# TtesseractT/Synthetic-Audio-Detection

Measured on AMD Instinct MI355X. Metric: 4s@32kHz segments/sec end-to-end (mel+ResNet+ensemble), 1/2/4/8 MI355X, higher is better.
Workload: dtype bf16; 1 GPU; end-to-end inference: B int16 4 s segments resident in HBM -> mel front end -> ResNet-18@512x512 -> 6 binary heads -> merge (+RCCL all-gather of logits); heads=6, distinct_backbones=1, micro_batch=2048, parallelism=dp1, frontend_overlapped=True

## Files before the change

synthetic-audio-detection_amd/csrc/halo256rs2.hip:

```cpp
#include "common.hpp"
#include "igemm.hpp"
#include "kernels.hpp"
#include "rwconv.hpp"

namespace sad {

namespace h44 {
constexpr int NW = 8, TC = 2;
constexpr int PW = 17, PITCH = PW * 128;
constexpr int NR[4] = {17, 17, 16, 16};
constexpr int NCV[4] = {17, 16, 17, 16};
constexpr int NP[4] = {37, 37, 34, 34};
constexpr int OFF[4] = {0, 37 * 1024, 74 * 1024, 108 * 1024};
constexpr int SMEM = 142 * 1024;
constexpr int BAD = 0x7FFFFFF0;
constexpr uint64_t KEY = 0x7929284ef1797ull;
static_assert(SMEM <= 160 * 1024, "LDS budget");
static_assert(16 * PITCH < 65536, "fragment row offsets are ds_read immediates");
constexpr int TPL[9] = {0, 0, 0, 0, 1, 1, 2, 2, 3};
constexpr int TRO[9] = {0, 0, 1, 1, 0, 1, 0, 0, 0};
constexpr int TCO[9] = {0, 1, 0, 1, 0, 0, 0, 1, 0};
constexpr int TAP[9] = {0, 2, 6, 8, 1, 7, 3, 5, 4};
constexpr int SCH[9][3] = {
    {1 | 3 << 3, 2 | 1 << 3, -1}, {1 | 4 << 3, 2 | 2 << 3, -1}, {2 | 3 << 3, 3 | 0 << 3, -1},
    {2 | 4 << 3, 3 | 1 << 3, -1}, {0 | 4 | 0 << 3, 3 | 2 << 3, -1}, {0 | 4 | 1 << 3, 3 | 3 << 3, -1},
    {0 | 4 | 2 << 3, 1 | 4 | 0 << 3, 3 | 4 << 3}, {0 | 4 | 3 << 3, 1 | 4 | 1 << 3, -1},
    {0 | 4 | 4 << 3, 1 | 4 | 2 << 3, 2 | 4 | 0 << 3}};
constexpr uint64_t pack_sch(int e) {
  uint64_t v = 0;
  for (int T = 0; T < 9; ++T) v |= (uint64_t)(SCH[T][e] < 0 ? 0x7F : SCH[T][e]) << (7 * T);
  return v;
}
constexpr uint64_t SCHP0 = pack_sch(0), SCHP1 = pack_sch(1), SCHP2 = pack_sch(2);
constexpr uint64_t pack_step() {
  uint64_t v = 0;
  for (int T = 0; T < 9; ++T) v |= (uint64_t)(TPL[T] | TRO[T] << 2 | TCO[T] << 3) << (4 * T);
  return v;
}
constexpr uint64_t STEPP = pack_step();
constexpr uint64_t pack_tap() {
  uint64_t v = 0;
  for (int T = 0; T < 8; ++T) v |= (uint64_t)TAP[T + 1] << (4 * T);
  return v;
}
constexpr uint64_t TAPP = pack_tap();
}

__device__ __forceinline__ int h44_key(int x) { return (int)((h44::KEY >> (3 * x)) & 7); }

typedef unsigned int h44_v4 __attribute__((ext_vector_type(4)));
typedef __bf16 h44_bf2 __attribute__((ext_vector_type(2)));
typedef float h44_f2 __attribute__((ext_vector_type(2)));
template <typename E = u16>
__device__ __forceinline__ uint32_t h44_pk(float lo, float hi) {
  if constexpr (is_f16_v<E>) return pk_f16(lo, hi);
  return __builtin_bit_cast(uint32_t, __builtin_convertvector((h44_f2){lo, hi}, h44_bf2));
}
__device__ __forceinline__ uint32_t h44_relu2(uint32_t x) {
  uint32_t r;
  asm("v_pk_max_i16 %0, %1, 0" : "=v"(r) : "v"(x));
  return r;
}

template <int BC, bool X3, typename E = u16>
__global__ __launch_bounds__(512, 1) void halo256rs2_kernel(BlockConvArgs a) {
  static_assert(!is_f16_v<E> || !X3, "fp16 has no split form");
  f16_kernel_entry<E>();
  using namespace h44;
  constexpr int NCG = BC / 32, NPG = NW / NCG, TP = 16 / NPG;
  static_assert(NCG * NPG == NW, "wave split");
  extern __shared__ __attribute__((aligned(16))) char smem[];
  const int tid = threadIdx.x, lane = tid & 63;
  const int wave = __builtin_amdgcn_readfirstlane(tid >> 6);
  const int fr = lane & 15, fg = lane >> 4;
  const int n_tc = a.Cout / BC;
  const int w = xcd_remap(blockIdx.x, gridDim.x);
  const int tc = w % n_tc;
  const int gp = gridDim.x / n_tc, wi = w / n_tc;
  const int tiles_x = a.Wo / 16, tiles_img = tiles_x * (a.Ho / 16);
  const int tiles_p = a.N * tiles_img;
  const int tp_begin = (int)((int64_t)wi * tiles_p / gp), tp_end = (int)((int64_t)(wi + 1) * tiles_p / gp);
  if (tp_begin >= tp_end) return;
  const int cgrp = wave % NCG, pgrp = wave / NCG;
  const int cw = tc * BC + cgrp * 16 * TC;
  const int r0w = pgrp * TP;
  const int ab = a.ablate;

  const int cinb = a.Cin * 2;
  const int nch = cinb / 128;
  const __amdgpu_buffer_rsrc_t r0 =
      __builtin_amdgcn_make_buffer_rsrc((void*)a.in0, (short)0, (int)a.in0_bytes, 0x00020000);
  const __amdgpu_buffer_rsrc_t rw =
      __builtin_amdgcn_make_buffer_rsrc((void*)a.wt, (short)0, (int)a.wt_bytes, 0x00020000);
  const int ps = (int)a.in0_pstride * 2;
  const unsigned lds0 = (unsigned)(uintptr_t)(__attribute__((address_space(3))) char*)smem;

  const int wrow = a.wt_ld * 2;
  const int wlane = (cw + fr) * wrow + fg * 16;
  auto load_w = [&](int kb, h44_v4 (&wv)[TC][2]) __attribute__((always_inline)) {
#pragma unroll
    for (int i = 0; i < TC; ++i)
#pragma unroll
      for (int h = 0; h < 2; ++h)
        wv[i][h] = __builtin_amdgcn_raw_buffer_load_b128(rw, wlane + i * 16 * wrow + h * 64,
                                                         __builtin_amdgcn_readfirstlane(kb), 0);
  };

  struct TileO {
    int b, iy0, ix0;
    bool ok;
  };
  auto tile_o = [&](int t) __attribute__((always_inline)) {
    const int tt = __builtin_amdgcn_readfirstlane(t);
    const int b = tt / tiles_img, rem = tt - b * tiles_img;
    const int ty = rem / tiles_x;
    return TileO{b, 32 * ty - 1, 32 * (rem - ty * tiles_x) - 1, tt < tp_end};
  };
  auto issue = [&](int P, const TileO& to, int c, int k) __attribute__((always_inline)) {
    const int q = wave + NW * k;
    const int np = P < 2 ? 37 : 34, nr = P < 2 ? 17 : 16, ncv = (P & 1) ? 16 : 17;
    if (q >= np || !to.ok) return;
    int ln;
    asm volatile("v_mov_b32 %0, %1" : "=v"(ln) : "v"(lane));
    const int u = 8 * q + (ln >> 3);
    const int r = (u * 3856) >> 16;
    const int x = u - PW * r;
    const int iy = to.iy0 + 2 * r + (P >> 1), ix = to.ix0 + 2 * x + (P & 1);
    const bool ok = r < nr && x < ncv && iy >= 0 && ix >= 0;
    const int off = ((to.b * a.H + iy) * a.W + ix) * ps + c * 128 + (((ln & 7) ^ h44_key(x)) << 4);
    const int poff = P == 0 ? OFF[0] : P == 1 ? OFF[1] : P == 2 ? OFF[2] : OFF[3];
    dma16_m0(r0, ok ? off : BAD, lds0 + poff + q * 1024);
  };

  {
    const TileO t0 = tile_o(tp_begin);
    for (int k = 0; k < 5; ++k) issue(0, t0, 0, k);
    for (int k = 0; k < 3; ++k) issue(1, t0, 0, k);
    issue(2, t0, 0, 0);
  }
  f32x4 biasv[TC];
#pragma unroll
  for (int i = 0; i < TC; ++i) biasv[i] = *(const f32x4*)(a.bias + cw + i * 16 + fg * 4);
  h44_v4 wcur[TC][2], wnxt[TC][2];
  load_w(0, wnxt);
  f32x4 acc[TC][TP];
#pragma unroll
  for (int i = 0; i < TC; ++i)
#pragma unroll
    for (int j = 0; j < TP; ++j) acc[i][j] = biasv[i];
  auto take_w = [&]() __attribute__((always_inline)) {
#pragma unroll
    for (int i = 0; i < TC; ++i)
#pragma unroll
      for (int h = 0; h < 2; ++h) wcur[i][h] = wnxt[i][h];
  };

  int lofs[2][2];
#pragma unroll
  for (int co = 0; co < 2; ++co)
#pragma unroll
    for (int h = 0; h < 2; ++h)
      lofs[co][h] = r0w * PITCH + (fr + co) * 128 + (((4 * h + fg) ^ h44_key(fr + co)) << 4);

  auto step = [&](int pbase, int co) __attribute__((always_inline)) {
    auto half = [&](auto hc) __attribute__((always_inline)) {
      constexpr int h = decltype(hc)::value;
      constexpr int NM = X3 && h == 0 ? 2 : 1;
      const char* pb = smem + pbase + (co ? lofs[1][h] : lofs[0][h]);
      uint4 bf[TP];
#pragma unroll
      for (int j = 0; j < TP; ++j) bf[j] = *(const uint4*)(pb + j * PITCH);
#pragma unroll
      for (int j = 0; j < TP; ++j)
#pragma unroll
        for (int m = 0; m < NM; ++m)
#pragma unroll
          for (int i = 0; i < TC; ++i)
            mfma_chunk<E>(__builtin_bit_cast(uint4, wcur[i][X3 ? m : h]), bf[j], acc[i][j]);
      __builtin_amdgcn_sched_group_barrier(0x100, 4, 0);
#pragma unroll
      for (int j = 0; j < TP - 4; ++j) {
        __builtin_amdgcn_sched_group_barrier(0x008, NM * TC, 0);
        __builtin_amdgcn_sched_group_barrier(0x100, 1, 0);
      }
      __builtin_amdgcn_sched_group_barrier(0x008, 4 * NM * TC, 0);
    };
    half(std::integral_constant<int, 0>{});
    half(std::integral_constant<int, 1>{});
  };

  auto epilogue = [&](int t) __attribute__((always_inline)) {
    const int b = t / tiles_img, rem = t - b * tiles_img;
    const int oy0 = (rem / tiles_x) * 16, ox0 = (rem - (rem / tiles_x) * tiles_x) * 16;
    u16* __restrict__ out = (u16*)a.out;
#pragma unroll
    for (int j = 0; j < TP; j += 2) {
      const int64_t px = (int64_t)(b * a.Ho + oy0 + r0w + j + (fg & 1)) * a.Wo + ox0 + fr;
#pragma unroll
      for (int i = 0; i < TC; ++i) {
        if constexpr (X3) {
          float v[2][4];
#pragma unroll
          for (int r = 0; r < 4; ++r) {
            v[0][r] = a.relu ? fmaxf(acc[i][j][r], 0.f) : acc[i][j][r];
            v[1][r] = a.relu ? fmaxf(acc[i][j + 1][r], 0.f) : acc[i][j + 1][r];
          }
          uint32_t qh[4], ql[4];
#pragma unroll
          for (int e = 0; e < 4; ++e) {
            const float x0 = v[e >> 1][2 * (e & 1)], x1 = v[e >> 1][2 * (e & 1) + 1];
            qh[e] = h44_pk(x0, x1);
            ql[e] = h44_pk(x0 - __uint_as_float(qh[e] << 16), x1 - __uint_as_float(qh[e] & 0xFFFF0000u));
          }
#pragma unroll
          for (int e = 0; e < 2; ++e) {
            const auto rh = __builtin_amdgcn_permlane16_swap(qh[e], qh[e + 2], false, false);
            qh[e] = rh[0];
            qh[e + 2] = rh[1];
            const auto rl = __builtin_amdgcn_permlane16_swap(ql[e], ql[e + 2], false, false);
            ql[e] = rl[0];
            ql[e + 2] = rl[1];
          }
          u16* op = out + px * a.out_pstride + 2 * cw + i * 16 + (fg >> 1) * 8;
          *(uint4*)op = make_uint4(qh[0], qh[1], qh[2], qh[3]);
          *(uint4*)(op + 32) = make_uint4(ql[0], ql[1], ql[2], ql[3]);
          continue;
        }
        const int co = cw + i * 16 + (fg >> 1) * 8;
        uint32_t q[4] = {h44_pk<E>(acc[i][j][0], acc[i][j][1]), h44_pk<E>(acc[i][j][2], acc[i][j][3]),
                         h44_pk<E>(acc[i][j + 1][0], acc[i][j + 1][1]), h44_pk<E>(acc[i][j + 1][2], acc[i][j + 1][3])};
        if (a.relu)
#pragma unroll
          for (int e = 0; e < 4; ++e) q[e] = h44_relu2(q[e]);
#pragma unroll
        for (int e = 0; e < 2; ++e) {
          const auto r = __builtin_amdgcn_permlane16_swap(q[e], q[e + 2], false, false);
          q[e] = r[0];
          q[e + 2] = r[1];
        }
        *(uint4*)(out + px * a.out_pstride + co) = make_uint4(q[0], q[1], q[2], q[3]);
      }
    }
#pragma unroll
    for (int i = 0; i < TC; ++i)
#pragma unroll
      for (int j = 0; j < TP; ++j) acc[i][j] = biasv[i];
  };

  bool post_epi = false;
  for (int t = tp_begin; t < tp_end; ++t) {
    const TileO tcur = tile_o(t), tnext = tile_o(t + 1);
    for (int c = 0; c < nch; ++c) {
      const int ncn = c + 1 < nch ? c + 1 : 0;
      const TileO& tn = c + 1 < nch ? tcur : tnext;
#pragma unroll 1
      for (int T = 0; T < 9; ++T) {
        if ((T == 0 || T == 4 || T == 6 || T == 8) && !(ab & 16)) {
          if (T == 0 && post_epi)
            asm volatile("s_waitcnt vmcnt(%0)" ::"n"((X3 ? 2 : 1) * TC * TP / 2) : "memory");
          else
            asm volatile("s_waitcnt vmcnt(0)" ::: "memory");
          post_epi = false;
          __builtin_amdgcn_s_barrier();
          asm volatile("" ::: "memory");
        }
        take_w();
        const int kbn = T < 8 ? (int)((TAPP >> (4 * T)) & 15) * cinb + c * 128 : ncn * 128;
        if (!(ab & 4)) load_w(kbn, wnxt);
        if (!(ab & 2)) {
#pragma unroll
          for (int e = 0; e < 3; ++e) {
            const uint64_t sp = e == 0 ? SCHP0 : e == 1 ? SCHP1 : SCHP2;
            const int d = (int)((sp >> (7 * T)) & 0x7F);
            if (d != 0x7F) {
              const bool nx = (d >> 2) & 1;
              issue(d & 3, nx ? tn : tcur, nx ? ncn : c, d >> 3);
            }
          }
        }
        const int sd = (int)((STEPP >> (4 * T)) & 15), pl = sd & 3;
        int co;
        asm volatile("s_lshr_b32 %0, %1, 3" : "=s"(co) : "s"(sd));
        step(1024 * (37 * pl - (pl == 3 ? 3 : 0)) + ((sd >> 2) & 1) * PITCH, co);
      }
    }
    if (!(ab & 8)) epilogue(t);
    post_epi = true;
  }
  asm volatile("s_waitcnt vmcnt(0)" ::: "memory");
}

template <int BC, bool X3, typename E = u16>
static int launch_halo256rs2_t(const BlockConvArgs& a, hipStream_t s) {
  using namespace h44;
  static bool attr = false;
  if (!attr) {
    SAD_CHECK_HIP(hipFuncSetAttribute((const void*)halo256rs2_kernel<BC, X3, E>,
                                      hipFuncAttributeMaxDynamicSharedMemorySize, SMEM));
    attr = true;
  }
  const int n_tc = a.Cout / BC;
  const int64_t tiles_p = (int64_t)a.N * (a.Ho / 16) * (a.Wo / 16);
  int64_t g = std::min<int64_t>(tiles_p * n_tc, 256);
  g = std::max<int64_t>(n_tc, g / n_tc * n_tc);
  hipLaunchKernelGGL((halo256rs2_kernel<BC, X3, E>), dim3((unsigned)g), dim3(512), SMEM, s, a);
  SAD_CHECK_HIP(hipGetLastError());
  return SAD_OK;
}

bool halo256rs2_ok(const BlockConvArgs& a) {
  return a.KH == 3 && a.KW == 3 && a.stride == 2 && a.pad == 1 && !a.in1 && !a.res && !a.st_part && !a.pool_out &&
         a.Cin % 64 == 0 && a.Cout % 128 == 0 && a.Ho % 16 == 0 && a.Wo % 16 == 0 && a.H == 2 * a.Ho &&
         a.W == 2 * a.Wo;
}

int launch_halo256rs2(const BlockConvArgs& a, hipStream_t s, bool x3, bool h16) {
  SAD_REQUIRE(!(x3 && h16), "variant 44: fp16 has no split form");
  SAD_REQUIRE(a.KH == 3 && a.KW == 3 && a.stride == 2 && a.pad == 1 && !a.in1 && !a.res && !a.st_part &&
                  !a.pool_out,
              "variant 44: 3x3/s2/p1, no shortcut / residual / pool / statistics");
  SAD_REQUIRE((a.Cin * 2) % 128 == 0 && a.Cout % 128 == 0, "variant 44: whole 128-B chunks, Cout % 128");
  SAD_REQUIRE(a.Ho % 16 == 0 && a.Wo % 16 == 0 && a.H == 2 * a.Ho && a.W == 2 * a.Wo,
              "variant 44: 16 x 16 output tiles, input exactly twice the output");
  SAD_REQUIRE(a.wt_ld >= 9 * a.Cin && (a.wt_ld * 2) % 16 == 0, "variant 44: weight rows");
  SAD_REQUIRE(a.out_pstride % 8 == 0 && a.in0_pstride % 8 == 0, "variant 44: pixel strides");
  SAD_REQUIRE(a.out != nullptr, "null output");
  SAD_REQUIRE(a.M == (int64_t)a.N * a.Ho * a.Wo, "variant 44: M = N Ho Wo");
  SAD_REQUIRE(((int64_t)a.N * a.H * a.W - 1) * a.in0_pstride * 2 + 2 * a.Cin < (1ll << 31) - 65536,
              "variant 44: input passes the 32-bit buffer range");
  if (h16)
    return a.Cout % 256 == 0 ? launch_halo256rs2_t<256, false, f16>(a, s) : launch_halo256rs2_t<128, false, f16>(a, s);
  if (x3)
    return a.Cout % 256 == 0 ? launch_halo256rs2_t<256, true>(a, s) : launch_halo256rs2_t<128, true>(a, s);
  return a.Cout % 256 == 0 ? launch_halo256rs2_t<256, false>(a, s) : launch_halo256rs2_t<128, false>(a, s);
}

}
```

synthetic-audio-detection_amd/csrc/l2s2conv.hip:

```cpp
#include "common.hpp"
#include "igemm.hpp"
#include "kernels.hpp"
#include "rwconv.hpp"

namespace sad {

namespace l2s {
constexpr int NW = 4;
constexpr int PRR = 17, PCW = 33;
constexpr int NEV = 9;
constexpr int PXB = 128;
constexpr int ROWB = PCW * PXB;
constexpr int ODDC = 17 * PXB;
constexpr int NPX = PRR * PCW;
constexpr int NDP = (NPX * PXB + 1023) / 1024;
constexpr int PATCH = NDP * 1024;
constexpr int QP = (NDP + NW - 1) / NW;
constexpr int OFF_BIAS = 2 * PATCH;
constexpr int SMEM = OFF_BIAS + 512;
constexpr int NS = 18;
constexpr int TP = 8;
constexpr int NUC = 9 * 2 * TP;
constexpr int DQ = 8;
constexpr int PDIV = 8;
constexpr int BAD = 0x7FFFFFF0;
constexpr uint64_t KEY = 0x7929284ef1797ull;
static_assert(SMEM <= 160 * 1024, "LDS budget");
static_assert(NUC / PDIV >= QP, "pieces fit the chunk's units");
static_assert(NW - 1 + NW * (QP - 2) < NDP, "only the last piece index can pass the patch");
static_assert(8 * ROWB + ODDC + 16 * PXB <= 65535, "fragment offsets are ds_read immediates");
}

__device__ __forceinline__ int l2s_key(int x) { return (int)((l2s::KEY >> (3 * x)) & 7); }

template <bool ST = false, typename E = u16>
__global__ __launch_bounds__(256, 1) void l2s2conv_kernel(BlockConvArgs a) {
  static_assert(!is_f16_v<E> || !ST, "the fused statistics are the bf16 trainer's");
  f16_kernel_entry<E>();
  using namespace l2s;
  const int ab = a.ablate;
  extern __shared__ __attribute__((aligned(16))) char smem[];
  const int tid = threadIdx.x, lane = tid & 63;
  const int wave = __builtin_amdgcn_readfirstlane(tid >> 6);
  const int fr = lane & 15, fg = lane >> 4;
  const int cw = wave * 32;
  const int w = xcd_remap(blockIdx.x, gridDim.x);
  const int tiles_x = a.Wo / 16, tiles_img = tiles_x * (a.Ho / 16);
  const int tiles_p = a.N * tiles_img;
  const int tp_begin = (int)((int64_t)w * tiles_p / gridDim.x), tp_end = (int)((int64_t)(w + 1) * tiles_p / gridDim.x);
  if (tp_begin >= tp_end) {
    if constexpr (ST) a.st_part[(int64_t)w * 256 + tid] = 0.f;
    return;
  }

  const __amdgpu_buffer_rsrc_t rx =
      __builtin_amdgcn_make_buffer_rsrc((void*)a.in0, (short)0, (int)a.in0_bytes, 0x00020000);
  const __amdgpu_buffer_rsrc_t ro =
      __builtin_amdgcn_make_buffer_rsrc((void*)a.out, (short)0, (int)a.out_bytes, 0x00020000);
  const unsigned lds0 = (unsigned)(uintptr_t)(__attribute__((address_space(3))) char*)smem;
  const int ps = (int)a.in0_pstride * 2;

  struct TileO {
    int base, b, oy0, ox0;
  };
  auto tile_o = [&](int t) __attribute__((always_inline)) {
    const int b = t / tiles_img, rem = t - b * tiles_img;
    const int ty = rem / tiles_x;
    TileO o;
    o.b = b;
    o.oy0 = ty * 16;
    o.ox0 = (rem - ty * tiles_x) * 16;
    o.base = ((b * a.H + 2 * o.oy0) * a.W + 2 * o.ox0) * ps;
    return o;
  };
  int prel[QP];
#pragma unroll
  for (int k = 0; k < QP; ++k) {
    const int u = 8 * (wave + NW * k) + (lane >> 3);
    const int r = (u * 1986) >> 16;
    const int cu = u - PCW * r;
    const int Y = r < NEV ? 2 * r : 2 * (r - NEV) + 1;
    const bool odd = cu >= 17;
    const int xp = odd ? cu - 17 : cu;
    const int X = 2 * xp + (odd ? 1 : 0);
    const int c = (lane & 7) ^ l2s_key(xp);
    prel[k] = (((Y - 1) * a.W + (X - 1)) * ps + (c << 4)) | (Y == 0 ? 1 : 0) | (X == 0 ? 2 : 0) | (u >= NPX ? 4 : 0);
  }
  const int hstep = 16 * a.W * ps;
  auto issue_piece = [&](int k, const TileO& o, int h) __attribute__((always_inline)) {
    const int q = wave + NW * k;
    if (k == QP - 1 && q >= NDP) return;
    const int mask = 4 | (h == 0 && o.oy0 == 0 ? 1 : 0) | (o.ox0 == 0 ? 2 : 0);
    const int e = prel[k];
    const int off = o.base + h * hstep + (e & ~15);
    dma16_m0(rx, (e & mask) ? BAD : off, lds0 + h * PATCH + q * 1024);
  };

  l1b_v4 wr[2][NS];
#pragma unroll
  for (int i = 0; i < 2; ++i)
#pragma unroll
    for (int s = 0; s < NS; ++s)
      wr[i][s] = *(const l1b_v4*)((const u16*)a.wt + (size_t)(cw + 16 * i + fr) * a.wt_ld + (s >> 1) * 64 +
                                  (s & 1) * 32 + fg * 8);
  if (tid < 32) *(float4*)(smem + OFF_BIAS + 16 * tid) = *(const float4*)(a.bias + 4 * tid);
  auto biasv = [&](int i) __attribute__((always_inline)) {
    return *(const f32x4*)(smem + OFF_BIAS + (cw + 16 * i + fg * 4) * 4);
  };
  {
    const TileO o0 = tile_o(tp_begin);
#pragma unroll
    for (int k = 0; k < QP; ++k) issue_piece(k, o0, 0);
  }
  asm volatile("s_waitcnt vmcnt(0)" ::: "memory");
  __syncthreads();
  f32x4 acc[2][TP];
#pragma unroll
  for (int i = 0; i < 2; ++i) {
    const f32x4 b0 = biasv(i);
#pragma unroll
    for (int j = 0; j < TP; ++j) acc[i][j] = b0;
  }

  int L[3][2];
#pragma unroll
  for (int kx = 0; kx < 3; ++kx) {
    const int xp = fr + (kx == 2 ? 1 : 0);
    const int key = l2s_key(xp);
#pragma unroll
    for (int kh = 0; kh < 2; ++kh) L[kx][kh] = (kx == 1 ? ODDC : 0) + xp * PXB + (((4 * kh + fg) ^ key) << 4);
  }

  float st_s[2][4] = {}, st_q[2][4] = {};
  for (int t = tp_begin; t < tp_end; ++t) {
    const TileO o = tile_o(t);
    const TileO onext = tile_o(t + 1 < tp_end ? t + 1 : t);
    const int frt = fr, fgt = fg;
    const int obase = ((o.b * a.Ho + o.oy0) * a.Wo + o.ox0) * (int)(a.out_pstride * 2);

    l1b_for<2>([&](auto hc) __attribute__((always_inline)) {
      constexpr int h = decltype(hc)::value;
      asm volatile("s_waitcnt vmcnt(8)" ::: "memory");
      __builtin_amdgcn_s_barrier();
      asm volatile("" ::: "memory");
      int B[3][2][2];
#pragma unroll
      for (int kx = 0; kx < 3; ++kx)
#pragma unroll
        for (int kh = 0; kh < 2; ++kh)
#pragma unroll
          for (int p = 0; p < 2; ++p) B[kx][kh][p] = L[kx][kh] + h * PATCH + p * NEV * ROWB;
      auto rd = [&](auto uc) __attribute__((always_inline)) -> uint4 {
        constexpr int u = decltype(uc)::value;
        constexpr int tap = u / 16, ky = tap / 3, kx = tap % 3, kh = (u / 8) & 1, j = u % 8;
        constexpr int p = ky == 1 ? 1 : 0, row = ky == 1 ? j : j + ky / 2;
        return *(const uint4*)(smem + B[kx][kh][p] + row * ROWB);
      };
      uint4 bq[DQ];
      l1b_for<DQ>([&](auto uc) __attribute__((always_inline)) { bq[decltype(uc)::value] = rd(uc); });
      l1b_for<NUC>([&](auto uc) __attribute__((always_inline)) {
        constexpr int u = decltype(uc)::value;
        constexpr int s = 2 * (u / 16) + ((u / 8) & 1), j = u % 8;
        const uint4 bf = bq[u % DQ];
        if constexpr (u + DQ < NUC) bq[u % DQ] = rd(std::integral_constant<int, u + DQ>{});
        if constexpr (u % PDIV == 0 && u / PDIV < QP) {
          if (ab & 32) {
          } else if constexpr (h == 0)
            issue_piece(u / PDIV, o, 1);
          else
            issue_piece(u / PDIV, onext, 0);
        }
        l1b_mfma_a<E>(acc[0][j], wr[0][s], bf);
        l1b_mfma_a<E>(acc[1][j], wr[1][s], bf);
      });
      __builtin_amdgcn_sched_barrier(0);
      asm volatile("s_nop 11" ::: "memory");
      __builtin_amdgcn_sched_barrier(0);

#pragma unroll
      for (int j = 0; j < TP; j += 2) {
#pragma unroll
        for (int i = 0; i < 2; ++i) {
          const f32x4 v0 = acc[i][j], v1 = acc[i][j + 1];
          if constexpr (ST) {
#pragma unroll
            for (int e = 0; e < 4; ++e) {
              st_s[i][e] += v0[e];
              st_s[i][e] += v1[e];
              st_q[i][e] = fmaf(v0[e], v0[e], st_q[i][e]);
              st_q[i][e] = fmaf(v1[e], v1[e], st_q[i][e]);
            }
          }
          uint32_t q[4] = {l1b_pk<E>(v0[0], v0[1]), l1b_pk<E>(v0[2], v0[3]), l1b_pk<E>(v1[0], v1[1]),
                           l1b_pk<E>(v1[2], v1[3])};
          if (a.relu)
#pragma unroll
            for (int e = 0; e < 4; ++e) q[e] = l1b_relu2(q[e]);
#pragma unroll
          for (int e = 0; e < 2; ++e) {
            const auto r = __builtin_amdgcn_permlane16_swap(q[e], q[e + 2], false, false);
            q[e] = r[0];
            q[e + 2] = r[1];
          }
          const int px = (8 * h + j + (fgt & 1)) * a.Wo + frt;
          const int co = cw + 16 * i + (fgt >> 1) * 8;
          if (!(ab & 8))
            __builtin_amdgcn_raw_buffer_store_b128(__builtin_bit_cast(l1b_v4, make_uint4(q[0], q[1], q[2], q[3])),
                                                   ro, px * (int)(a.out_pstride * 2) + co * 2, obase, 0);
          const f32x4 b0 = biasv(i);
          acc[i][j] = b0;
          acc[i][j + 1] = b0;
        }
      }
    });
  }
  if constexpr (ST) {
#pragma unroll
    for (int i = 0; i < 2; ++i)
#pragma unroll
      for (int e = 0; e < 4; ++e)
#pragma unroll
        for (int off = 1; off < 16; off <<= 1) {
          st_s[i][e] += __shfl_xor(st_s[i][e], off, 64);
          st_q[i][e] += __shfl_xor(st_q[i][e], off, 64);
        }
    if (fr == 0) {
#pragma unroll
      for (int i = 0; i < 2; ++i)
#pragma unroll
        for (int e = 0; e < 4; ++e) {
          const int c = cw + 16 * i + 4 * fg + e;
          a.st_part[(int64_t)w * 256 + c] = st_s[i][e];
          a.st_part[(int64_t)w * 256 + 128 + c] = st_q[i][e];
        }
    }
  }
  asm volatile("s_waitcnt vmcnt(0)" ::: "memory");
}

int launch_l2s2conv(const BlockConvArgs& a, hipStream_t s, bool h16) {
  using namespace l2s;
  SAD_REQUIRE(a.KH == 3 && a.KW == 3 && a.stride == 2 && a.pad == 1 && !a.in1 && !a.res && !a.pool_out,
              "variant 43: 3x3/s2/p1, no shortcut, residual or pool");
  SAD_REQUIRE(!a.st_part || (!a.relu && a.st_rows), "variant 43 statistics: the raw conv (no ReLU), st_rows set");
  SAD_REQUIRE(a.Cin == 64 && a.Cout == 128, "variant 43: Cin 64, Cout 128");
  SAD_REQUIRE(a.Ho % 16 == 0 && a.Wo % 16 == 0 && a.H == 2 * a.Ho && a.W == 2 * a.Wo,
              "variant 43: output must tile by 16 x 16, input twice its size");
  SAD_REQUIRE(a.wt_ld >= 9 * 64 && a.wt_ld % 8 == 0, "variant 43: weight rows");
  SAD_REQUIRE(a.in0_pstride % 8 == 0 && a.in0_pstride >= 64 && a.out_pstride % 8 == 0 && a.out_pstride >= 128 && a.out,
              "variant 43: 16-B aligned pixel strides, an output");
  const int64_t tiles = (int64_t)a.N * (a.Ho / 16) * (a.Wo / 16);
  if (tiles == 0) return SAD_OK;
  const int64_t g = std::min<int64_t>(tiles, 256);
  BlockConvArgs b = a;
  b.out_bytes = ((int64_t)a.N * a.Ho * a.Wo - 1) * a.out_pstride * 2 + 256;
  SAD_REQUIRE(b.out_bytes < (1ll << 31) - 65536, "variant 43: output passes the 32-bit buffer range");
  if (h16) {
    SAD_REQUIRE(!a.st_part, "variant 43: no fused statistics in fp16");
    static bool attr = false;
    if (!attr) {
      SAD_CHECK_HIP(hipFuncSetAttribute((const void*)l2s2conv_kernel<false, f16>,
                                        hipFuncAttributeMaxDynamicSharedMemorySize, SMEM));
      attr = true;
    }
    hipLaunchKernelGGL((l2s2conv_kernel<false, f16>), dim3((unsigned)g), dim3(256), SMEM, s, b);
  } else if (a.st_part) {
    static bool attr = false;
    if (!attr) {
      SAD_CHECK_HIP(hipFuncSetAttribute((const void*)l2s2conv_kernel<true>, hipFuncAttributeMaxDynamicSharedMemorySize, SMEM));
      attr = true;
    }
    hipLaunchKernelGGL(l2s2conv_kernel<true>, dim3((unsigned)g), dim3(256), SMEM, s, b);
    *a.st_rows = (int)g;
  } else {
    static bool attr = false;
    if (!attr) {
      SAD_CHECK_HIP(hipFuncSetAttribute((const void*)l2s2conv_kernel<false>, hipFuncAttributeMaxDynamicSharedMemorySize, SMEM));
      attr = true;
    }
    hipLaunchKernelGGL(l2s2conv_kernel<false>, dim3((unsigned)g), dim3(256), SMEM, s, b);
  }
  SAD_CHECK_HIP(hipGetLastError());
  return SAD_OK;
}

}
```

Baseline: 64550 segments/s.

## Precompute halo DMA offsets in LDS tables and fully unroll tap schedule

The stride-2 halo conv kernels now compute per-lane DMA offsets and edge masks once into a small LDS table. Per-plane bases and masks are hoisted per tile, and the 9-tap loop with its load schedule is fully unrolled at compile time. Tile coordinates advance incrementally instead of through divisions, weights are double-buffered by register set instead of copied, and ablation checks move into a separate kernel so the production path drops them. The l2s kernel also interleaves epilogue stores and bias folding into the MFMA stream. The aim is to cut scalar and vector address arithmetic and branches in the inner loop, at the cost of code size, register pressure and added LDS.

New measurement: 64970 segments/s, median of 6. About the same (+0.7%).

```diff
diff --git a/synthetic-audio-detection_amd/csrc/halo256rs2.hip b/synthetic-audio-detection_amd/csrc/halo256rs2.hip
--- a/synthetic-audio-detection_amd/csrc/halo256rs2.hip
+++ b/synthetic-audio-detection_amd/csrc/halo256rs2.hip
@@ -12,11 +12,16 @@
 constexpr int NCV[4] = {17, 16, 17, 16};
 constexpr int NP[4] = {37, 37, 34, 34};
 constexpr int OFF[4] = {0, 37 * 1024, 74 * 1024, 108 * 1024};
-constexpr int SMEM = 142 * 1024;
+constexpr int PLANES = 142 * 1024;
+constexpr int NK = 5;
+constexpr int DUMMY = PLANES + NW * NK * 256;
+constexpr int SMEM = DUMMY + 1024;
+constexpr int ESH = 27;
 constexpr int BAD = 0x7FFFFFF0;
 constexpr uint64_t KEY = 0x7929284ef1797ull;
 static_assert(SMEM <= 160 * 1024, "LDS budget");
 static_assert(16 * PITCH < 65536, "fragment row offsets are ds_read immediates");
+static_assert(NW * (NK - 1) < NP[3] && NW * NK >= NP[0], "only the last piece index can pass a plane");
 constexpr int TPL[9] = {0, 0, 0, 0, 1, 1, 2, 2, 3};
 constexpr int TRO[9] = {0, 0, 1, 1, 0, 1, 0, 0, 0};
 constexpr int TCO[9] = {0, 1, 0, 1, 0, 0, 0, 1, 0};
@@ -26,24 +31,18 @@
     {2 | 4 << 3, 3 | 1 << 3, -1}, {0 | 4 | 0 << 3, 3 | 2 << 3, -1}, {0 | 4 | 1 << 3, 3 | 3 << 3, -1},
     {0 | 4 | 2 << 3, 1 | 4 | 0 << 3, 3 | 4 << 3}, {0 | 4 | 3 << 3, 1 | 4 | 1 << 3, -1},
     {0 | 4 | 4 << 3, 1 | 4 | 2 << 3, 2 | 4 | 0 << 3}};
-constexpr uint64_t pack_sch(int e) {
-  uint64_t v = 0;
-  for (int T = 0; T < 9; ++T) v |= (uint64_t)(SCH[T][e] < 0 ? 0x7F : SCH[T][e]) << (7 * T);
-  return v;
-}
-constexpr uint64_t SCHP0 = pack_sch(0), SCHP1 = pack_sch(1), SCHP2 = pack_sch(2);
-constexpr uint64_t pack_step() {
-  uint64_t v = 0;
-  for (int T = 0; T < 9; ++T) v |= (uint64_t)(TPL[T] | TRO[T] << 2 | TCO[T] << 3) << (4 * T);
-  return v;
-}
-constexpr uint64_t STEPP = pack_step();
-constexpr uint64_t pack_tap() {
-  uint64_t v = 0;
-  for (int T = 0; T < 8; ++T) v |= (uint64_t)TAP[T + 1] << (4 * T);
-  return v;
-}
-constexpr uint64_t TAPP = pack_tap();
+constexpr int sch_next_k(int T, int e) {
+  int t = T, i = e + 1;
+  for (;;) {
+    if (i == 3) {
+      i = 0;
+      t = (t + 1) % 9;
+    }
+    if (SCH[t][i] >= 0) return SCH[t][i] >> 3;
+    ++i;
+  }
+}
+constexpr int SCH_K0 = SCH[0][0] >> 3;
 }
 
 __device__ __forceinline__ int h44_key(int x) { return (int)((h44::KEY >> (3 * x)) & 7); }
@@ -56,15 +55,11 @@
   if constexpr (is_f16_v<E>) return pk_f16(lo, hi);
   return __builtin_bit_cast(uint32_t, __builtin_convertvector((h44_f2){lo, hi}, h44_bf2));
 }
-__device__ __forceinline__ uint32_t h44_relu2(uint32_t x) {
-  uint32_t r;
-  asm("v_pk_max_i16 %0, %1, 0" : "=v"(r) : "v"(x));
-  return r;
-}
-
-template <int BC, bool X3, typename E = u16>
-__global__ __launch_bounds__(512, 1) void halo256rs2_kernel(BlockConvArgs a) {
+
+template <int BC, bool X3, bool AB, typename E>
+__device__ __forceinline__ void halo256rs2_body(const BlockConvArgs& a) {
   static_assert(!is_f16_v<E> || !X3, "fp16 has no split form");
+  static_assert(!AB || (!X3 && !is_f16_v<E>), "ablations: the bf16 form");
   f16_kernel_entry<E>();
   using namespace h44;
   constexpr int NCG = BC / 32, NPG = NW / NCG, TP = 16 / NPG;
@@ -84,14 +79,14 @@
   const int cgrp = wave % NCG, pgrp = wave / NCG;
   const int cw = tc * BC + cgrp * 16 * TC;
   const int r0w = pgrp * TP;
-  const int ab = a.ablate;
+  const int ab = AB ? a.ablate : 0;
 
   const int cinb = a.Cin * 2;
   const int nch = cinb / 128;
-  const __amdgpu_buffer_rsrc_t r0 =
-      __builtin_amdgcn_make_buffer_rsrc((void*)a.in0, (short)0, (int)a.in0_bytes, 0x00020000);
+  l1b_v4 rx = {(unsigned)(uintptr_t)a.in0, (unsigned)((uintptr_t)a.in0 >> 32) & 0xFFFFu, (unsigned)a.in0_bytes, 0x00020000u};
+  asm volatile("" : "+s"(rx));
   const __amdgpu_buffer_rsrc_t rw =
-      __builtin_amdgcn_make_buffer_rsrc((void*)a.wt, (short)0, (int)a.wt_bytes, 0x00020000);
+      __builtin_amdgcn_make_buffer_rsrc((void*)a.wt, (short)0, (ab & 4) ? 0 : (int)a.wt_bytes, 0x00020000);
   const int ps = (int)a.in0_pstride * 2;
   const unsigned lds0 = (unsigned)(uintptr_t)(__attribute__((address_space(3))) char*)smem;
 
@@ -102,58 +97,97 @@
     for (int i = 0; i < TC; ++i)
 #pragma unroll
       for (int h = 0; h < 2; ++h)
-        wv[i][h] = __builtin_amdgcn_raw_buffer_load_b128(rw, wlane + i * 16 * wrow + h * 64,
-                                                         __builtin_amdgcn_readfirstlane(kb), 0);
+        wv[i][h] = __builtin_amdgcn_raw_buffer_load_b128(rw, wlane + h * 64,
+                                                         __builtin_amdgcn_readfirstlane(kb + i * 16 * wrow), 0);
   };
 
   struct TileO {
-    int b, iy0, ix0;
+    int base, opix, oy0, ox0;
     bool ok;
   };
   auto tile_o = [&](int t) __attribute__((always_inline)) {
     const int tt = __builtin_amdgcn_readfirstlane(t);
     const int b = tt / tiles_img, rem = tt - b * tiles_img;
     const int ty = rem / tiles_x;
-    return TileO{b, 32 * ty - 1, 32 * (rem - ty * tiles_x) - 1, tt < tp_end};
-  };
-  auto issue = [&](int P, const TileO& to, int c, int k) __attribute__((always_inline)) {
-    const int q = wave + NW * k;
-    const int np = P < 2 ? 37 : 34, nr = P < 2 ? 17 : 16, ncv = (P & 1) ? 16 : 17;
-    if (q >= np || !to.ok) return;
-    int ln;
-    asm volatile("v_mov_b32 %0, %1" : "=v"(ln) : "v"(lane));
-    const int u = 8 * q + (ln >> 3);
+    TileO o;
+    o.oy0 = ty * 16;
+    o.ox0 = (rem - ty * tiles_x) * 16;
+    o.base = ((b * a.H + 2 * o.oy0 - 1) * a.W + 2 * o.ox0 - 1) * ps;
+    o.opix = (b * a.Ho + o.oy0) * a.Wo + o.ox0;
+    o.ok = true;
+    return o;
+  };
+  const int wrap_i = 31 * a.W * ps, wrap_o = 15 * a.Wo;
+  auto tile_step = [&](const TileO& o, bool ok) __attribute__((always_inline)) {
+    TileO n;
+    n.ox0 = o.ox0 + 16;
+    n.oy0 = o.oy0;
+    n.base = o.base + 32 * ps;
+    n.opix = o.opix + 16;
+    if (n.ox0 == a.Wo) {
+      n.ox0 = 0;
+      n.oy0 += 16;
+      n.base += wrap_i;
+      n.opix += wrap_o;
+      if (n.oy0 == a.Ho) n.oy0 = 0;
+    }
+    n.ok = ok;
+    return n;
+  };
+
+  int* const tab = (int*)(smem + PLANES) + wave * (NK * 64) + lane;
+  auto piece_entry = [&](int k) __attribute__((always_inline)) {
+    const int u = 8 * (wave + NW * k) + (lane >> 3);
     const int r = (u * 3856) >> 16;
     const int x = u - PW * r;
-    const int iy = to.iy0 + 2 * r + (P >> 1), ix = to.ix0 + 2 * x + (P & 1);
-    const bool ok = r < nr && x < ncv && iy >= 0 && ix >= 0;
-    const int off = ((to.b * a.H + iy) * a.W + ix) * ps + c * 128 + (((ln & 7) ^ h44_key(x)) << 4);
-    const int poff = P == 0 ? OFF[0] : P == 1 ? OFF[1] : P == 2 ? OFF[2] : OFF[3];
-    dma16_m0(r0, ok ? off : BAD, lds0 + poff + q * 1024);
-  };
-
+    const int edge = (r >= 17 ? 1 : 0) | (r == 0 ? 2 : 0) | (x == 0 ? 4 : 0) | (r == 16 ? 8 : 0) | (x == 16 ? 16 : 0);
+    const unsigned off = (unsigned)((2 * r * a.W + 2 * x) * ps + (((lane & 7) ^ h44_key(x)) << 4)) >> 4;
+    return (int)(((unsigned)edge << ESH) | (off & ((1u << ESH) - 1)));
+  };
+  auto plane_base = [&](const TileO& o, int P, int c) __attribute__((always_inline)) {
+    return o.base + ((P >> 1) * a.W + (P & 1)) * ps + c * 128;
+  };
+  auto plane_mask = [&](const TileO& o, int P, bool loop = true) __attribute__((always_inline)) {
+    const unsigned m = 1u | ((P >> 1) == 0 && o.oy0 == 0 ? 2u : 0u) | ((P & 1) == 0 && o.ox0 == 0 ? 4u : 0u) |
+                       ((P >> 1) ? 8u : 0u) | ((P & 1) ? 16u : 0u);
+    return o.ok && !(loop && (ab & 2)) ? (int)(m << ESH) : -1;
+  };
+  const unsigned dstw = __builtin_amdgcn_readfirstlane(lds0 + wave * 1024);
+  auto piece = [&](auto Pc, auto kc, int e, int pbase, int pmask) __attribute__((always_inline)) {
+    constexpr int P = decltype(Pc)::value, k = decltype(kc)::value;
+    if constexpr (NW * k + NW - 1 >= NP[P]) {
+      const bool has = wave + NW * k < NP[P];
+      l1b_dma16<0>(rx, (e & (has ? pmask : -1)) ? BAD : pbase + (int)((unsigned)e << 4),
+                   has ? dstw + (OFF[P] + k * NW * 1024) : lds0 + DUMMY);
+    } else {
+      l1b_dma16<OFF[P] + k * NW * 1024>(rx, (e & pmask) ? BAD : pbase + (int)((unsigned)e << 4), dstw);
+    }
+  };
+
+  TileO tcur = tile_o(tp_begin);
   {
-    const TileO t0 = tile_o(tp_begin);
-    for (int k = 0; k < 5; ++k) issue(0, t0, 0, k);
-    for (int k = 0; k < 3; ++k) issue(1, t0, 0, k);
-    issue(2, t0, 0, 0);
+    const int b0 = plane_base(tcur, 0, 0), m0 = plane_mask(tcur, 0, false);
+    const int b1 = plane_base(tcur, 1, 0), m1 = plane_mask(tcur, 1, false);
+    const int b2 = plane_base(tcur, 2, 0), m2 = plane_mask(tcur, 2, false);
+    l1b_for<NK>([&](auto kc) __attribute__((always_inline)) {
+      constexpr int k = decltype(kc)::value;
+      const int e = piece_entry(k);
+      tab[64 * k] = e;
+      piece(std::integral_constant<int, 0>{}, kc, e, b0, m0);
+      if constexpr (k < 3) piece(std::integral_constant<int, 1>{}, kc, e, b1, m1);
+      if constexpr (k < 1) piece(std::integral_constant<int, 2>{}, kc, e, b2, m2);
+    });
   }
   f32x4 biasv[TC];
 #pragma unroll
   for (int i = 0; i < TC; ++i) biasv[i] = *(const f32x4*)(a.bias + cw + i * 16 + fg * 4);
-  h44_v4 wcur[TC][2], wnxt[TC][2];
-  load_w(0, wnxt);
+  h44_v4 wset[2][TC][2];
+  load_w(0, wset[1]);
   f32x4 acc[TC][TP];
 #pragma unroll
   for (int i = 0; i < TC; ++i)
 #pragma unroll
     for (int j = 0; j < TP; ++j) acc[i][j] = biasv[i];
-  auto take_w = [&]() __attribute__((always_inline)) {
-#pragma unroll
-    for (int i = 0; i < TC; ++i)
-#pragma unroll
-      for (int h = 0; h < 2; ++h) wcur[i][h] = wnxt[i][h];
-  };
 
   int lofs[2][2];
 #pragma unroll
@@ -162,21 +196,25 @@
     for (int h = 0; h < 2; ++h)
       lofs[co][h] = r0w * PITCH + (fr + co) * 128 + (((4 * h + fg) ^ h44_key(fr + co)) << 4);
 
-  auto step = [&](int pbase, int co) __attribute__((always_inline)) {
+  auto step = [&](auto Tc, const h44_v4 (&wv)[TC][2]) __attribute__((always_inline)) {
+    constexpr int T = decltype(Tc)::value;
     auto half = [&](auto hc) __attribute__((always_inline)) {
       constexpr int h = decltype(hc)::value;
       constexpr int NM = X3 && h == 0 ? 2 : 1;
-      const char* pb = smem + pbase + (co ? lofs[1][h] : lofs[0][h]);
+      unsigned po;
+      asm volatile("v_add_u32 %0, %1, %2" : "=v"(po) : "s"(lds0 + OFF[TPL[T]]), "v"(lofs[TCO[T]][h]));
+      const auto* pb = (const __attribute__((address_space(3))) char*)(uintptr_t)po + TRO[T] * PITCH;
       uint4 bf[TP];
 #pragma unroll
-      for (int j = 0; j < TP; ++j) bf[j] = *(const uint4*)(pb + j * PITCH);
-#pragma unroll
       for (int j = 0; j < TP; ++j)
+        bf[j] = __builtin_bit_cast(uint4, *(const __attribute__((address_space(3))) h44_v4*)(pb + j * PITCH));
+#pragma unroll
+      for (int j = 0; j < TP; ++j)
 #pragma unroll
         for (int m = 0; m < NM; ++m)
 #pragma unroll
           for (int i = 0; i < TC; ++i)
-            mfma_chunk<E>(__builtin_bit_cast(uint4, wcur[i][X3 ? m : h]), bf[j], acc[i][j]);
+            mfma_chunk<E>(__builtin_bit_cast(uint4, wv[i][X3 ? m : h]), bf[j], acc[i][j]);
       __builtin_amdgcn_sched_group_barrier(0x100, 4, 0);
 #pragma unroll
       for (int j = 0; j < TP - 4; ++j) {
@@ -189,13 +227,15 @@
     half(std::integral_constant<int, 1>{});
   };
 
-  auto epilogue = [&](int t) __attribute__((always_inline)) {
-    const int b = t / tiles_img, rem = t - b * tiles_img;
-    const int oy0 = (rem / tiles_x) * 16, ox0 = (rem - (rem / tiles_x) * tiles_x) * 16;
+  const int rl = a.relu ? 0 : (int)0x80008000u;
+  auto epilogue = [&](const TileO& o) __attribute__((always_inline)) {
+    int el;
+    asm volatile("v_mov_b32 %0, %1" : "=v"(el) : "v"(lane));
+    const int fr = el & 15, fg = el >> 4;
     u16* __restrict__ out = (u16*)a.out;
 #pragma unroll
     for (int j = 0; j < TP; j += 2) {
-      const int64_t px = (int64_t)(b * a.Ho + oy0 + r0w + j + (fg & 1)) * a.Wo + ox0 + fr;
+      const int64_t px = (int64_t)o.opix + (r0w + j + (fg & 1)) * a.Wo + fr;
 #pragma unroll
       for (int i = 0; i < TC; ++i) {
         if constexpr (X3) {
@@ -217,9 +257,9 @@
             const auto rh = __builtin_amdgcn_permlane16_swap(qh[e], qh[e + 2], false, false);
             qh[e] = rh[0];
             qh[e + 2] = rh[1];
-            const auto rl = __builtin_amdgcn_permlane16_swap(ql[e], ql[e + 2], false, false);
-            ql[e] = rl[0];
-            ql[e + 2] = rl[1];
+            const auto rl2 = __builtin_amdgcn_permlane16_swap(ql[e], ql[e + 2], false, false);
+            ql[e] = rl2[0];
+            ql[e + 2] = rl2[1];
           }
           u16* op = out + px * a.out_pstride + 2 * cw + i * 16 + (fg >> 1) * 8;
           *(uint4*)op = make_uint4(qh[0], qh[1], qh[2], qh[3]);
@@ -229,9 +269,8 @@
         const int co = cw + i * 16 + (fg >> 1) * 8;
         uint32_t q[4] = {h44_pk<E>(acc[i][j][0], acc[i][j][1]), h44_pk<E>(acc[i][j][2], acc[i][j][3]),
                          h44_pk<E>(acc[i][j + 1][0], acc[i][j + 1][1]), h44_pk<E>(acc[i][j + 1][2], acc[i][j + 1][3])};
-        if (a.relu)
-#pragma unroll
-          for (int e = 0; e < 4; ++e) q[e] = h44_relu2(q[e]);
+#pragma unroll
+        for (int e = 0; e < 4; ++e) q[e] = l1b_relu2s(q[e], rl);
 #pragma unroll
         for (int e = 0; e < 2; ++e) {
           const auto r = __builtin_amdgcn_permlane16_swap(q[e], q[e + 2], false, false);
@@ -247,65 +286,99 @@
       for (int j = 0; j < TP; ++j) acc[i][j] = biasv[i];
   };
 
+  int pe = tab[64 * SCH_K0];
   bool post_epi = false;
   for (int t = tp_begin; t < tp_end; ++t) {
-    const TileO tcur = tile_o(t), tnext = tile_o(t + 1);
+    const TileO tnext = tile_step(tcur, t + 1 < tp_end);
     for (int c = 0; c < nch; ++c) {
-      const int ncn = c + 1 < nch ? c + 1 : 0;
-      const TileO& tn = c + 1 < nch ? tcur : tnext;
-#pragma unroll 1
-      for (int T = 0; T < 9; ++T) {
-        if ((T == 0 || T == 4 || T == 6 || T == 8) && !(ab & 16)) {
-          if (T == 0 && post_epi)
-            asm volatile("s_waitcnt vmcnt(%0)" ::"n"((X3 ? 2 : 1) * TC * TP / 2) : "memory");
-          else
-            asm volatile("s_waitcnt vmcnt(0)" ::: "memory");
-          post_epi = false;
-          __builtin_amdgcn_s_barrier();
-          asm volatile("" ::: "memory");
-        }
-        take_w();
-        const int kbn = T < 8 ? (int)((TAPP >> (4 * T)) & 15) * cinb + c * 128 : ncn * 128;
-        if (!(ab & 4)) load_w(kbn, wnxt);
-        if (!(ab & 2)) {
-#pragma unroll
-          for (int e = 0; e < 3; ++e) {
-            const uint64_t sp = e == 0 ? SCHP0 : e == 1 ? SCHP1 : SCHP2;
-            const int d = (int)((sp >> (7 * T)) & 0x7F);
-            if (d != 0x7F) {
-              const bool nx = (d >> 2) & 1;
-              issue(d & 3, nx ? tn : tcur, nx ? ncn : c, d >> 3);
+      const bool last = c + 1 == nch;
+      const int ncn = last ? 0 : c + 1;
+      const int nbase = last ? tnext.base : tcur.base, noy0 = last ? tnext.oy0 : tcur.oy0,
+                nox0 = last ? tnext.ox0 : tcur.ox0;
+      const TileO tn = {nbase, 0, noy0, nox0, last ? tnext.ok : true};
+      const int pb[2][4] = {{0, plane_base(tcur, 1, c), plane_base(tcur, 2, c), plane_base(tcur, 3, c)},
+                            {plane_base(tn, 0, ncn), plane_base(tn, 1, ncn), plane_base(tn, 2, ncn), 0}};
+      const int pm[2][4] = {{0, plane_mask(tcur, 1), plane_mask(tcur, 2), plane_mask(tcur, 3)},
+                            {plane_mask(tn, 0), plane_mask(tn, 1), plane_mask(tn, 2), 0}};
+      const int kbn0 = ncn * 128;
+      l1b_for<9>([&](auto Tc) __attribute__((always_inline)) {
+        constexpr int T = decltype(Tc)::value;
+        if constexpr (T == 0 || T == 4 || T == 6 || T == 8) {
+          if (!(ab & 16)) {
+            if constexpr (T == 0) {
+              if (post_epi)
+                asm volatile("s_waitcnt vmcnt(%0)" ::"n"((X3 ? 2 : 1) * TC * TP / 2) : "memory");
+              else
+                asm volatile("s_waitcnt vmcnt(0)" ::: "memory");
+              post_epi = false;
+            } else {
+              asm volatile("s_waitcnt vmcnt(0)" ::: "memory");
             }
+            __builtin_amdgcn_s_barrier();
+            asm volatile("" ::: "memory");
           }
         }
-        const int sd = (int)((STEPP >> (4 * T)) & 15), pl = sd & 3;
-        int co;
-        asm volatile("s_lshr_b32 %0, %1, 3" : "=s"(co) : "s"(sd));
-        step(1024 * (37 * pl - (pl == 3 ? 3 : 0)) + ((sd >> 2) & 1) * PITCH, co);
-      }
+        if constexpr (T == 0) {
+#pragma unroll
+          for (int i = 0; i < TC; ++i)
+#pragma unroll
+            for (int h = 0; h < 2; ++h) wset[0][i][h] = wset[1][i][h];
+        } else {
+          __builtin_amdgcn_sched_barrier(0);
+        }
+        load_w(T < 8 ? TAP[T < 8 ? T + 1 : 0] * cinb + c * 128 : kbn0, wset[(T + 1) & 1]);
+        l1b_for<3>([&](auto ec) __attribute__((always_inline)) {
+          constexpr int e = decltype(ec)::value, d = SCH[T][e];
+          if constexpr (d >= 0) {
+            constexpr int P = d & 3, nx = (d >> 2) & 1, k = d >> 3, kn = sch_next_k(T, e);
+            piece(std::integral_constant<int, P>{}, std::integral_constant<int, k>{}, pe, pb[nx][P], pm[nx][P]);
+            pe = tab[64 * kn];
+          }
+        });
+        __builtin_amdgcn_sched_barrier(0);
+        step(Tc, wset[T & 1]);
+      });
     }
-    if (!(ab & 8)) epilogue(t);
+    if (!(ab & 8)) epilogue(tcur);
     post_epi = true;
+    tcur = tnext;
   }
   asm volatile("s_waitcnt vmcnt(0)" ::: "memory");
 }
 
 template <int BC, bool X3, typename E = u16>
-static int launch_halo256rs2_t(const BlockConvArgs& a, hipStream_t s) {
+__global__ __launch_bounds__(512, 1) void halo256rs2_kernel(BlockConvArgs a) {
+  halo256rs2_body<BC, X3, false, E>(a);
+}
+template <int BC>
+__global__ __launch_bounds__(512, 1) void halo256rs2_ablate_kernel(BlockConvArgs a) {
+  halo256rs2_body<BC, false, true, u16>(a);
+}
+
+template <typename K>
+static int launch_halo256rs2_k(K kern, bool& attr, int BC, const BlockConvArgs& a, hipStream_t s) {
   using namespace h44;
-  static bool attr = false;
   if (!attr) {
-    SAD_CHECK_HIP(hipFuncSetAttribute((const void*)halo256rs2_kernel<BC, X3, E>,
-                                      hipFuncAttributeMaxDynamicSharedMemorySize, SMEM));
+    SAD_CHECK_HIP(hipFuncSetAttribute((const void*)kern, hipFuncAttributeMaxDynamicSharedMemorySize, SMEM));
     attr = true;
   }
   const int n_tc = a.Cout / BC;
   const int64_t tiles_p = (int64_t)a.N * (a.Ho / 16) * (a.Wo / 16);
   int64_t g = std::min<int64_t>(tiles_p * n_tc, 256);
   g = std::max<int64_t>(n_tc, g / n_tc * n_tc);
-  hipLaunchKernelGGL((halo256rs2_kernel<BC, X3, E>), dim3((unsigned)g), dim3(512), SMEM, s, a);
+  hipLaunchKernelGGL(kern, dim3((unsigned)g), dim3(512), SMEM, s, a);
   SAD_CHECK_HIP(hipGetLastError());
   return SAD_OK;
+}
+template <int BC, bool X3, typename E = u16>
+static int launch_halo256rs2_t(const BlockConvArgs& a, hipStream_t s) {
+  static bool attr = false;
+  return launch_halo256rs2_k(halo256rs2_kernel<BC, X3, E>, attr, BC, a, s);
+}
+template <int BC>
+static int launch_halo256rs2_ablate_t(const BlockConvArgs& a, hipStream_t s) {
+  static bool attr = false;
+  return launch_halo256rs2_k(halo256rs2_ablate_kernel<BC>, attr, BC, a, s);
 }
 
 bool halo256rs2_ok(const BlockConvArgs& a) {
@@ -328,6 +401,8 @@
   SAD_REQUIRE(a.M == (int64_t)a.N * a.Ho * a.Wo, "variant 44: M = N Ho Wo");
   SAD_REQUIRE(((int64_t)a.N * a.H * a.W - 1) * a.in0_pstride * 2 + 2 * a.Cin < (1ll << 31) - 65536,
               "variant 44: input passes the 32-bit buffer range");
+  SAD_REQUIRE(!a.ablate || (!x3 && !h16), "variant 44 ablations: the bf16 form");
+  if (a.ablate) return a.Cout % 256 == 0 ? launch_halo256rs2_ablate_t<256>(a, s) : launch_halo256rs2_ablate_t<128>(a, s);
   if (h16)
     return a.Cout % 256 == 0 ? launch_halo256rs2_t<256, false, f16>(a, s) : launch_halo256rs2_t<128, false, f16>(a, s);
   if (x3)
diff --git a/synthetic-audio-detection_amd/csrc/l2s2conv.hip b/synthetic-audio-detection_amd/csrc/l2s2conv.hip
--- a/synthetic-audio-detection_amd/csrc/l2s2conv.hip
+++ b/synthetic-audio-detection_amd/csrc/l2s2conv.hip
@@ -20,12 +20,26 @@
 constexpr int SMEM = OFF_BIAS + 512;
 constexpr int NS = 18;
 constexpr int TP = 8;
-constexpr int NUC = 9 * 2 * TP;
+constexpr int NUC = NS * TP;
 constexpr int DQ = 8;
 constexpr int PDIV = 8;
 constexpr int BAD = 0x7FFFFFF0;
 constexpr uint64_t KEY = 0x7929284ef1797ull;
+constexpr int ESH = 27;
+constexpr int SA = 4, NB = NS - SA;
+constexpr int unit_s(int u) { return u < SA * TP ? u / TP : SA + (u - SA * TP) % NB; }
+constexpr int unit_j(int u) { return u < SA * TP ? u % TP : (u - SA * TP) / NB; }
+constexpr int EQ0 = 3, EQ1 = 8;
+static_assert(2 * (EQ0 + 1) >= 6 && EQ0 < EQ1 && EQ1 < NB, "epilogue parts sit >= 6 MFMAs behind their rows' last MFMA");
+constexpr int stores_behind_last_piece() {
+  int n = 2;
+  for (int j = 2; j < TP; ++j)
+    if (SA * TP + j * NB + EQ1 >= (QP - 1) * PDIV) ++n;
+  return n;
+}
+constexpr int NSB = stores_behind_last_piece();
 static_assert(SMEM <= 160 * 1024, "LDS budget");
+static_assert(SMEM + NW * QP * 256 > 160 * 1024, "the piece table would fit LDS: move it there");
 static_assert(NUC / PDIV >= QP, "pieces fit the chunk's units");
 static_assert(NW - 1 + NW * (QP - 2) < NDP, "only the last piece index can pass the patch");
 static_assert(8 * ROWB + ODDC + 16 * PXB <= 65535, "fragment offsets are ds_read immediates");
@@ -33,12 +47,13 @@
 
 __device__ __forceinline__ int l2s_key(int x) { return (int)((l2s::KEY >> (3 * x)) & 7); }
 
-template <bool ST = false, typename E = u16>
-__global__ __launch_bounds__(256, 1) void l2s2conv_kernel(BlockConvArgs a) {
-  static_assert(!is_f16_v<E> || !ST, "the fused statistics are the bf16 trainer's");
+template <bool ST, bool AB, typename E>
+__device__ __forceinline__ void l2s2conv_body(const BlockConvArgs& a) {
+  static_assert(!is_f16_v<E> || (!ST && !AB), "fp16: the plain inference form");
+  static_assert(!(ST && AB), "ablations: the bf16 inference form");
   f16_kernel_entry<E>();
   using namespace l2s;
-  const int ab = a.ablate;
+  const int ab = AB ? a.ablate : 0;
   extern __shared__ __attribute__((aligned(16))) char smem[];
   const int tid = threadIdx.x, lane = tid & 63;
   const int wave = __builtin_amdgcn_readfirstlane(tid >> 6);
@@ -53,26 +68,45 @@
     return;
   }
 
-  const __amdgpu_buffer_rsrc_t rx =
-      __builtin_amdgcn_make_buffer_rsrc((void*)a.in0, (short)0, (int)a.in0_bytes, 0x00020000);
+  l1b_v4 rx = {(unsigned)(uintptr_t)a.in0, (unsigned)((uintptr_t)a.in0 >> 32) & 0xFFFFu, (unsigned)a.in0_bytes, 0x00020000u};
+  asm volatile("" : "+s"(rx));
   const __amdgpu_buffer_rsrc_t ro =
       __builtin_amdgcn_make_buffer_rsrc((void*)a.out, (short)0, (int)a.out_bytes, 0x00020000);
   const unsigned lds0 = (unsigned)(uintptr_t)(__attribute__((address_space(3))) char*)smem;
   const int ps = (int)a.in0_pstride * 2;
+  const int pso = (int)a.out_pstride * 2;
+  const int orow = a.Wo * pso;
 
   struct TileO {
-    int base, b, oy0, ox0;
+    int base, obase, oy0, ox0;
   };
   auto tile_o = [&](int t) __attribute__((always_inline)) {
     const int b = t / tiles_img, rem = t - b * tiles_img;
     const int ty = rem / tiles_x;
     TileO o;
-    o.b = b;
     o.oy0 = ty * 16;
     o.ox0 = (rem - ty * tiles_x) * 16;
     o.base = ((b * a.H + 2 * o.oy0) * a.W + 2 * o.ox0) * ps;
+    o.obase = ((b * a.Ho + o.oy0) * a.Wo + o.ox0) * pso;
     return o;
   };
+  const int wrap_i = 31 * a.W * ps, wrap_o = 15 * orow;
+  auto tile_step = [&](const TileO& o) __attribute__((always_inline)) {
+    TileO n;
+    n.ox0 = o.ox0 + 16;
+    n.oy0 = o.oy0;
+    n.base = o.base + 32 * ps;
+    n.obase = o.obase + 16 * pso;
+    if (n.ox0 == a.Wo) {
+      n.ox0 = 0;
+      n.oy0 += 16;
+      n.base += wrap_i;
+      n.obase += wrap_o;
+      if (n.oy0 == a.Ho) n.oy0 = 0;
+    }
+    return n;
+  };
+
   int prel[QP];
 #pragma unroll
   for (int k = 0; k < QP; ++k) {
@@ -84,16 +118,24 @@
     const int xp = odd ? cu - 17 : cu;
     const int X = 2 * xp + (odd ? 1 : 0);
     const int c = (lane & 7) ^ l2s_key(xp);
-    prel[k] = (((Y - 1) * a.W + (X - 1)) * ps + (c << 4)) | (Y == 0 ? 1 : 0) | (X == 0 ? 2 : 0) | (u >= NPX ? 4 : 0);
+    const int edge = (u >= NPX ? 1 : 0) | (Y == 0 ? 2 : 0) | (X == 0 ? 4 : 0);
+    const unsigned off = (unsigned)((Y * a.W + X) * ps + (c << 4)) >> 4;
+    prel[k] = (int)(((unsigned)edge << ESH) | (off & ((1u << ESH) - 1)));
   }
   const int hstep = 16 * a.W * ps;
-  auto issue_piece = [&](int k, const TileO& o, int h) __attribute__((always_inline)) {
-    const int q = wave + NW * k;
-    if (k == QP - 1 && q >= NDP) return;
-    const int mask = 4 | (h == 0 && o.oy0 == 0 ? 1 : 0) | (o.ox0 == 0 ? 2 : 0);
+  auto patch_base = [&](const TileO& o, int h) __attribute__((always_inline)) {
+    return o.base - (a.W + 1) * ps + h * hstep;
+  };
+  auto patch_mask = [&](const TileO& o, int h) __attribute__((always_inline)) {
+    return (int)((unsigned)(1 | (h == 0 && o.oy0 == 0 ? 2 : 0) | (o.ox0 == 0 ? 4 : 0)) << ESH);
+  };
+  const unsigned dstw = __builtin_amdgcn_readfirstlane(lds0 + wave * 1024);
+  auto issue_piece = [&](auto kc, auto hc, int pbase, int pmask) __attribute__((always_inline)) {
+    constexpr int k = decltype(kc)::value, h = decltype(hc)::value;
+    if constexpr (NW * k + NW - 1 >= NDP)
+      if (wave + NW * k >= NDP) return;
     const int e = prel[k];
-    const int off = o.base + h * hstep + (e & ~15);
-    dma16_m0(rx, (e & mask) ? BAD : off, lds0 + h * PATCH + q * 1024);
+    l1b_dma16<h * PATCH + k * NW * 1024>(rx, (e & pmask) ? BAD : pbase + (int)((unsigned)e << 4), dstw);
   };
 
   l1b_v4 wr[2][NS];
@@ -104,23 +146,16 @@
       wr[i][s] = *(const l1b_v4*)((const u16*)a.wt + (size_t)(cw + 16 * i + fr) * a.wt_ld + (s >> 1) * 64 +
                                   (s & 1) * 32 + fg * 8);
   if (tid < 32) *(float4*)(smem + OFF_BIAS + 16 * tid) = *(const float4*)(a.bias + 4 * tid);
-  auto biasv = [&](int i) __attribute__((always_inline)) {
-    return *(const f32x4*)(smem + OFF_BIAS + (cw + 16 * i + fg * 4) * 4);
-  };
+  TileO ocur = tile_o(tp_begin);
   {
-    const TileO o0 = tile_o(tp_begin);
-#pragma unroll
-    for (int k = 0; k < QP; ++k) issue_piece(k, o0, 0);
+    const int pb = patch_base(ocur, 0), pm = patch_mask(ocur, 0);
+    l1b_for<QP>([&](auto kc) __attribute__((always_inline)) { issue_piece(kc, std::integral_constant<int, 0>{}, pb, pm); });
   }
   asm volatile("s_waitcnt vmcnt(0)" ::: "memory");
   __syncthreads();
-  f32x4 acc[2][TP];
-#pragma unroll
-  for (int i = 0; i < 2; ++i) {
-    const f32x4 b0 = biasv(i);
-#pragma unroll
-    for (int j = 0; j < TP; ++j) acc[i][j] = b0;
-  }
+  f32x4 bv[2];
+#pragma unroll
+  for (int i = 0; i < 2; ++i) bv[i] = *(const f32x4*)(smem + OFF_BIAS + (cw + 16 * i + fg * 4) * 4);
 
   int L[3][2];
 #pragma unroll
@@ -130,17 +165,21 @@
 #pragma unroll
     for (int kh = 0; kh < 2; ++kh) L[kx][kh] = (kx == 1 ? ODDC : 0) + xp * PXB + (((4 * kh + fg) ^ key) << 4);
   }
+  const int OV = ((fg & 1) * a.Wo + fr) * pso + (cw + (fg >> 1) * 8) * 2;
+  const int rl = a.relu ? 0 : (int)0x80008000u;
 
   float st_s[2][4] = {}, st_q[2][4] = {};
+  f32x4 acc[2][TP];
   for (int t = tp_begin; t < tp_end; ++t) {
-    const TileO o = tile_o(t);
-    const TileO onext = tile_o(t + 1 < tp_end ? t + 1 : t);
-    const int frt = fr, fgt = fg;
-    const int obase = ((o.b * a.Ho + o.oy0) * a.Wo + o.ox0) * (int)(a.out_pstride * 2);
+    const TileO ostep = tile_step(ocur);
+    const TileO onext = t + 1 < tp_end ? ostep : ocur;
+    const TileO o = ocur;
+    const int pb1 = patch_base(o, 1), pm1 = patch_mask(o, 1);
+    const int pb0n = patch_base(onext, 0), pm0n = patch_mask(onext, 0);
 
     l1b_for<2>([&](auto hc) __attribute__((always_inline)) {
       constexpr int h = decltype(hc)::value;
-      asm volatile("s_waitcnt vmcnt(8)" ::: "memory");
+      asm volatile("s_waitcnt vmcnt(%0)" ::"n"(NSB) : "memory");
       __builtin_amdgcn_s_barrier();
       asm volatile("" ::: "memory");
       int B[3][2][2];
@@ -152,36 +191,17 @@
           for (int p = 0; p < 2; ++p) B[kx][kh][p] = L[kx][kh] + h * PATCH + p * NEV * ROWB;
       auto rd = [&](auto uc) __attribute__((always_inline)) -> uint4 {
         constexpr int u = decltype(uc)::value;
-        constexpr int tap = u / 16, ky = tap / 3, kx = tap % 3, kh = (u / 8) & 1, j = u % 8;
+        constexpr int s = unit_s(u), j = unit_j(u);
+        constexpr int tap = s >> 1, ky = tap / 3, kx = tap % 3, kh = s & 1;
         constexpr int p = ky == 1 ? 1 : 0, row = ky == 1 ? j : j + ky / 2;
         return *(const uint4*)(smem + B[kx][kh][p] + row * ROWB);
       };
-      uint4 bq[DQ];
-      l1b_for<DQ>([&](auto uc) __attribute__((always_inline)) { bq[decltype(uc)::value] = rd(uc); });
-      l1b_for<NUC>([&](auto uc) __attribute__((always_inline)) {
-        constexpr int u = decltype(uc)::value;
-        constexpr int s = 2 * (u / 16) + ((u / 8) & 1), j = u % 8;
-        const uint4 bf = bq[u % DQ];
-        if constexpr (u + DQ < NUC) bq[u % DQ] = rd(std::integral_constant<int, u + DQ>{});
-        if constexpr (u % PDIV == 0 && u / PDIV < QP) {
-          if (ab & 32) {
-          } else if constexpr (h == 0)
-            issue_piece(u / PDIV, o, 1);
-          else
-            issue_piece(u / PDIV, onext, 0);
-        }
-        l1b_mfma_a<E>(acc[0][j], wr[0][s], bf);
-        l1b_mfma_a<E>(acc[1][j], wr[1][s], bf);
-      });
-      __builtin_amdgcn_sched_barrier(0);
-      asm volatile("s_nop 11" ::: "memory");
-      __builtin_amdgcn_sched_barrier(0);
-
-#pragma unroll
-      for (int j = 0; j < TP; j += 2) {
-#pragma unroll
-        for (int i = 0; i < 2; ++i) {
-          const f32x4 v0 = acc[i][j], v1 = acc[i][j + 1];
+      const int osh = o.obase + 8 * h * orow;
+      uint32_t eq0 = 0, eq2 = 0;
+      auto epi = [&](auto jc, auto pc) __attribute__((always_inline)) {
+        constexpr int j = decltype(jc)::value, part = decltype(pc)::value, i = part >> 1;
+        const f32x4 v0 = acc[i][j], v1 = acc[i][j + 1];
+        if constexpr ((part & 1) == 0) {
           if constexpr (ST) {
 #pragma unroll
             for (int e = 0; e < 4; ++e) {
@@ -191,28 +211,59 @@
               st_q[i][e] = fmaf(v1[e], v1[e], st_q[i][e]);
             }
           }
-          uint32_t q[4] = {l1b_pk<E>(v0[0], v0[1]), l1b_pk<E>(v0[2], v0[3]), l1b_pk<E>(v1[0], v1[1]),
-                           l1b_pk<E>(v1[2], v1[3])};
-          if (a.relu)
-#pragma unroll
-            for (int e = 0; e < 4; ++e) q[e] = l1b_relu2(q[e]);
-#pragma unroll
-          for (int e = 0; e < 2; ++e) {
-            const auto r = __builtin_amdgcn_permlane16_swap(q[e], q[e + 2], false, false);
-            q[e] = r[0];
-            q[e + 2] = r[1];
+          uint32_t q0 = l1b_pk<E>(v0[0], v0[1]), q2 = l1b_pk<E>(v1[0], v1[1]);
+          if constexpr (!ST) {
+            q0 = l1b_relu2s(q0, rl);
+            q2 = l1b_relu2s(q2, rl);
           }
-          const int px = (8 * h + j + (fgt & 1)) * a.Wo + frt;
-          const int co = cw + 16 * i + (fgt >> 1) * 8;
+          const auto r = __builtin_amdgcn_permlane16_swap(q0, q2, false, false);
+          eq0 = r[0];
+          eq2 = r[1];
+        } else {
+          uint32_t q1 = l1b_pk<E>(v0[2], v0[3]), q3 = l1b_pk<E>(v1[2], v1[3]);
+          if constexpr (!ST) {
+            q1 = l1b_relu2s(q1, rl);
+            q3 = l1b_relu2s(q3, rl);
+          }
+          const auto r = __builtin_amdgcn_permlane16_swap(q1, q3, false, false);
           if (!(ab & 8))
-            __builtin_amdgcn_raw_buffer_store_b128(__builtin_bit_cast(l1b_v4, make_uint4(q[0], q[1], q[2], q[3])),
-                                                   ro, px * (int)(a.out_pstride * 2) + co * 2, obase, 0);
-          const f32x4 b0 = biasv(i);
-          acc[i][j] = b0;
-          acc[i][j + 1] = b0;
-        }
-      }
+            __builtin_amdgcn_raw_buffer_store_b128((l1b_v4){eq0, r[0], eq2, r[1]}, ro, OV + 32 * i, osh + j * orow, 0);
+        }
+      };
+      uint4 bq[DQ];
+      l1b_for<DQ>([&](auto uc) __attribute__((always_inline)) { bq[decltype(uc)::value] = rd(uc); });
+      l1b_for<NUC>([&](auto uc) __attribute__((always_inline)) {
+        constexpr int u = decltype(uc)::value;
+        constexpr int s = unit_s(u), j = unit_j(u);
+        const uint4 bf = bq[u % DQ];
+        if constexpr (u + DQ < NUC) bq[u % DQ] = rd(std::integral_constant<int, u + DQ>{});
+        if constexpr (u % PDIV == 0 && u / PDIV < QP) {
+          if (!(ab & 32))
+            issue_piece(std::integral_constant<int, u / PDIV>{}, std::integral_constant<int, h ^ 1>{}, h == 0 ? pb1 : pb0n,
+                        h == 0 ? pm1 : pm0n);
+        }
+        if constexpr (s == 0) {
+          l1b_mfma_ac<E>(acc[0][j], wr[0][s], bf, bv[0]);
+          l1b_mfma_ac<E>(acc[1][j], wr[1][s], bf, bv[1]);
+        } else {
+          l1b_mfma_a<E>(acc[0][j], wr[0][s], bf);
+          l1b_mfma_a<E>(acc[1][j], wr[1][s], bf);
+        }
+        if constexpr (u >= SA * TP && j >= 2) {
+          constexpr int q = (u - SA * TP) % NB;
+          if constexpr (q == EQ0 || q == EQ1) {
+            __builtin_amdgcn_sched_barrier(0);
+            epi(std::integral_constant<int, (j & ~1) - 2>{}, std::integral_constant<int, 2 * (j & 1) + (q == EQ1 ? 1 : 0)>{});
+            __builtin_amdgcn_sched_barrier(0);
+          }
+        }
+      });
+      __builtin_amdgcn_sched_barrier(0);
+      asm volatile("s_nop 11" ::: "memory");
+      __builtin_amdgcn_sched_barrier(0);
+      l1b_for<4>([&](auto pc) __attribute__((always_inline)) { epi(std::integral_constant<int, TP - 2>{}, pc); });
     });
+    ocur = ostep;
   }
   if constexpr (ST) {
 #pragma unroll
@@ -236,6 +287,14 @@
     }
   }
   asm volatile("s_waitcnt vmcnt(0)" ::: "memory");
+}
+
+template <bool ST = false, typename E = u16>
+__global__ __launch_bounds__(256, 1) void l2s2conv_kernel(BlockConvArgs a) {
+  l2s2conv_body<ST, false, E>(a);
+}
+__global__ __launch_bounds__(256, 1) void l2s2conv_ablate_kernel(BlockConvArgs a) {
+  l2s2conv_body<false, true, u16>(a);
 }
 
 int launch_l2s2conv(const BlockConvArgs& a, hipStream_t s, bool h16) {
@@ -243,43 +302,40 @@
   SAD_REQUIRE(a.KH == 3 && a.KW == 3 && a.stride == 2 && a.pad == 1 && !a.in1 && !a.res && !a.pool_out,
               "variant 43: 3x3/s2/p1, no shortcut, residual or pool");
   SAD_REQUIRE(!a.st_part || (!a.relu && a.st_rows), "variant 43 statistics: the raw conv (no ReLU), st_rows set");
+  SAD_REQUIRE(!a.ablate || (!h16 && !a.st_part), "variant 43 ablations: the bf16 inference form");
   SAD_REQUIRE(a.Cin == 64 && a.Cout == 128, "variant 43: Cin 64, Cout 128");
   SAD_REQUIRE(a.Ho % 16 == 0 && a.Wo % 16 == 0 && a.H == 2 * a.Ho && a.W == 2 * a.Wo,
               "variant 43: output must tile by 16 x 16, input twice its size");
   SAD_REQUIRE(a.wt_ld >= 9 * 64 && a.wt_ld % 8 == 0, "variant 43: weight rows");
   SAD_REQUIRE(a.in0_pstride % 8 == 0 && a.in0_pstride >= 64 && a.out_pstride % 8 == 0 && a.out_pstride >= 128 && a.out,
               "variant 43: 16-B aligned pixel strides, an output");
+  SAD_REQUIRE(a.in0_bytes < (1ll << 31) - 65536, "variant 43: input passes the 32-bit buffer range");
   const int64_t tiles = (int64_t)a.N * (a.Ho / 16) * (a.Wo / 16);
   if (tiles == 0) return SAD_OK;
   const int64_t g = std::min<int64_t>(tiles, 256);
   BlockConvArgs b = a;
   b.out_bytes = ((int64_t)a.N * a.Ho * a.Wo - 1) * a.out_pstride * 2 + 256;
   SAD_REQUIRE(b.out_bytes < (1ll << 31) - 65536, "variant 43: output passes the 32-bit buffer range");
+  auto go = [&](auto kern, bool& attr) {
+    if (!attr) {
+      SAD_CHECK_HIP(hipFuncSetAttribute((const void*)kern, hipFuncAttributeMaxDynamicSharedMemorySize, SMEM));
+      attr = true;
+    }
+    hipLaunchKernelGGL(kern, dim3((unsigned)g), dim3(256), SMEM, s, b);
+    return SAD_OK;
+  };
+  static bool attr[4] = {};
+  int rc;
   if (h16) {
     SAD_REQUIRE(!a.st_part, "variant 43: no fused statistics in fp16");
-    static bool attr = false;
-    if (!attr) {
-      SAD_CHECK_HIP(hipFuncSetAttribute((const void*)l2s2conv_kernel<false, f16>,
-                                        hipFuncAttributeMaxDynamicSharedMemorySize, SMEM));
-      attr = true;
-    }
-    hipLaunchKernelGGL((l2s2conv_kernel<false, f16>), dim3((unsigned)g), dim3(256), SMEM, s, b);
+    rc = go(l2s2conv_kernel<false, f16>, attr[0]);
   } else if (a.st_part) {
-    static bool attr = false;
-    if (!attr) {
-      SAD_CHECK_HIP(hipFuncSetAttribute((const void*)l2s2conv_kernel<true>, hipFuncAttributeMaxDynamicSharedMemorySize, SMEM));
-      attr = true;
-    }
-    hipLaunchKernelGGL(l2s2conv_kernel<true>, dim3((unsigned)g), dim3(256), SMEM, s, b);
-    *a.st_rows = (int)g;
+    rc = go(l2s2conv_kernel<true>, attr[1]);
+    if (rc == SAD_OK) *a.st_rows = (int)g;
   } else {
-    static bool attr = false;
-    if (!attr) {
-      SAD_CHECK_HIP(hipFuncSetAttribute((const void*)l2s2conv_kernel<false>, hipFuncAttributeMaxDynamicSharedMemorySize, SMEM));
-      attr = true;
-    }
-    hipLaunchKernelGGL(l2s2conv_kernel<false>, dim3((unsigned)g), dim3(256), SMEM, s, b);
-  }
+    rc = a.ablate ? go(l2s2conv_ablate_kernel, attr[3]) : go(l2s2conv_kernel<false>, attr[2]);
+  }
+  if (rc != SAD_OK) return rc;
   SAD_CHECK_HIP(hipGetLastError());
   return SAD_OK;
 }
```
